# Exidekat/TransformerUpscaler

Hardware: AMD Instinct MI355X
Metric: images/sec, FastTransformer 2x 720p->1080p inference (higher is better)
Workload: dtype bf16

## Files before the change

transformerupscaler_amd/csrc/block_stream.hip:

```cpp
#include "common.h"
#include <stdlib.h>
#include <type_traits>
#include <utility>

namespace {

typedef __attribute__((ext_vector_type(16))) float f32x16;

constexpr int BS_NT = 512;
constexpr int TILE = 12288;
constexpr int L_TAB = 0;
constexpr int L_A = 8192, L_WQK = L_A, L_WV = L_A + 2 * TILE;
constexpr int L_B = L_A + 4 * TILE;
constexpr int L_KX = L_B, L_VX = L_B + 16384;
constexpr int L_OF = L_B + 32768;
constexpr int BS_LDS = L_OF + 65536;
constexpr int CHUNK = 2 * TILE;
static_assert(BS_LDS <= 163840, "LDS");
static_assert(L_A + 6 * CHUNK <= BS_LDS && L_A + 3 * CHUNK >= L_B + 2 * TILE, "MLP ring: six slots; slots 3-5 (the first chunks) clear of the proj tiles");
constexpr int T_QKB = 0, T_B1 = 384, T_BP = 1152, T_B2 = 1344;
constexpr int PROJ_T[6] = {L_WV, L_WQK, L_WV + TILE, L_WQK + TILE, L_B, L_B + TILE};

struct StreamBlock { const char* wqk; const char* wv; const char* wproj; const char* w1; const char* w2; const float* tab; const float* sbias; };
template <int PAR_, bool F1_, bool GE_, bool F2_, bool DM_> struct MlpSlot {
    static constexpr int PAR = PAR_, NM = (F1_ && F2_) ? 24 : 12;
    static constexpr bool F1 = F1_, GE = GE_, F2 = F2_, DM = DM_;
    static constexpr bool LNS = !F1_ && !GE_ && F2_;
};
constexpr int BS_MAX_BLK = 8;
struct StreamTable { StreamBlock b[BS_MAX_BLK]; };

template <class F, int... I> TUP_DEVICE void static_for_impl(F&& f, std::integer_sequence<int, I...>) { (f(std::integral_constant<int, I>{}), ...); }
template <int N, class F> TUP_DEVICE void static_for(F&& f) { static_for_impl(f, std::make_integer_sequence<int, N>{}); }

TUP_DEVICE f32x16 mfma32(bf16x8 a, bf16x8 b, f32x16 c) { return __builtin_amdgcn_mfma_f32_32x32x16_bf16(a, b, c, 0, 0, 0); }
TUP_DEVICE f32x16 mfma32h(bf16x8 a, bf16x8 b, f32x16 c) {
    return __builtin_amdgcn_mfma_f32_32x32x16_f16(__builtin_bit_cast(h8, a), __builtin_bit_cast(h8, b), c, 0, 0, 0);
}
#define FENCE() __builtin_amdgcn_sched_barrier(0)

TUP_DEVICE void lds_write_b128(uint32_t addr, bf16x8 v) { asm volatile("ds_write_b128 %0, %1" ::"v"(addr), "v"(v) : "memory"); }
TUP_DEVICE void lds_write_b128_off(uint32_t addr, bf16x8 v, int off) { asm volatile("ds_write_b128 %0, %1 offset:%2" ::"v"(addr), "v"(v), "i"(off) : "memory"); }
TUP_DEVICE void lds_write_b32(uint32_t addr, float v) { asm volatile("ds_write_b32 %0, %1" ::"v"(addr), "v"(v) : "memory"); }
TUP_DEVICE uint32_t lds_read_b32_off(uint32_t addr, int off) {
    uint32_t v;
    asm volatile("ds_read_b32 %0, %1 offset:%2" : "=v"(v) : "v"(addr), "i"(off));
    return v;
}
TUP_DEVICE f32x4 lds_read_f4_off(uint32_t addr, int off) { return __builtin_bit_cast(f32x4, lds_read_b128_asm_off(addr, off)); }
template <int N> TUP_DEVICE void vm_wait() { asm volatile("s_waitcnt vmcnt(%0)" ::"n"(N) : "memory"); }
TUP_DEVICE void barrier_all() {
    asm volatile("s_waitcnt vmcnt(0) lgkmcnt(0)\n\ts_barrier" ::: "memory");
}

TUP_DEVICE __amdgpu_buffer_rsrc_t bs_rsrc(const void* p) { return __builtin_amdgcn_make_buffer_rsrc(const_cast<void*>(p), 0, 0x7fffffff, 0x00020000); }
TUP_DEVICE void bs_dma(__amdgpu_buffer_rsrc_t r, char* lds_dst, uint32_t lane16, int soff) {
    __builtin_amdgcn_raw_ptr_buffer_load_lds(r, (__attribute__((address_space(3))) void*)lds_dst, 16, (int)lane16, soff, 0, 0);
}

#pragma clang diagnostic push
#pragma clang diagnostic ignored "-Winline-asm"
template <int OFF> TUP_DEVICE void bs_dma_on(__amdgpu_buffer_rsrc_t rs, uint32_t lds_base, uint32_t lane16, uint32_t soff) {
    static_assert(OFF >= 0 && OFF < 4096, "12-bit immediate offset");
    asm volatile("s_bitcmp1_b32 %0, 31\n\ts_cbranch_scc1 1f\n\ts_mov_b32 m0, %0\n\ts_nop 0\n\tbuffer_load_dwordx4 %1, %2, %3 offen offset:%4 lds\n1:"
                 :: "s"(lds_base), "v"(lane16), "s"(rs), "s"(soff), "n"(OFF) : "memory", "scc", "m0");
}
#pragma clang diagnostic pop

TUP_DEVICE bf16x8 pack8(float a0, float a1, float a2, float a3, float a4, float a5, float a6, float a7) {
    return __builtin_bit_cast(bf16x8, u32x4{pack_bf16x2(a0, a1), pack_bf16x2(a2, a3), pack_bf16x2(a4, a5), pack_bf16x2(a6, a7)});
}
template <int O> TUP_DEVICE bf16x8 pack8_regs(const f32x16& v) { return pack8(v[O], v[O + 1], v[O + 2], v[O + 3], v[O + 4], v[O + 5], v[O + 6], v[O + 7]); }
TUP_DEVICE float half_sum(float v) {
    const uint32_t u = __builtin_bit_cast(uint32_t, v);
    const auto q = __builtin_amdgcn_permlane32_swap(u, u, false, false);
    return __builtin_bit_cast(float, q[0]) + __builtin_bit_cast(float, opaque_copy(q[1]));
}
TUP_DEVICE float half_max(float v) {
    const uint32_t u = __builtin_bit_cast(uint32_t, v);
    const auto q = __builtin_amdgcn_permlane32_swap(u, u, false, false);
    return vmax(__builtin_bit_cast(float, q[0]), __builtin_bit_cast(float, opaque_copy(q[1])));
}
TUP_DEVICE float max3(float a, float b, float c) { return __builtin_fmaxf(__builtin_fmaxf(a, b), c); }

struct LnStats { float s[2], q[2]; };
TUP_DEVICE void ln_stats_tile(LnStats& st, const f32x16& t) {
#pragma unroll
    for (int i = 0; i < 16; ++i) { st.s[i & 1] += t[i]; st.q[i & 1] = __builtin_fmaf(t[i], t[i], st.q[i & 1]); }
}
template <int K> TUP_DEVICE void ln_stats_op(LnStats& st, const f32x16& t) {
    constexpr int i = K >> 1;
    if constexpr ((K & 1) == 0) { st.s[i & 1] += t[i]; asm volatile("" : "+v"(st.s[i & 1])); }
    else { st.q[i & 1] = __builtin_fmaf(t[i], t[i], st.q[i & 1]); asm volatile("" : "+v"(st.q[i & 1])); }
}
template <int K0, int K1> TUP_DEVICE void ln_stats_ops(LnStats& st, const f32x16& t) {
    static_for<(K1 > K0 ? K1 - K0 : 0)>([&](auto k) { ln_stats_op<K0 + decltype(k)::value>(st, t); });
}
TUP_DEVICE void ln_finish(const LnStats& st, float& rstd, float& shift) {
    const float sum = half_sum(st.s[0] + st.s[1]), sq = half_sum(st.q[0] + st.q[1]);
    const float mean = sum * (1.0f / 192);
    rstd = rsqrtf(fmaxf(__builtin_fmaf(-mean, mean, sq * (1.0f / 192)), 0.f) + 1e-5f);
    shift = -mean * rstd;
}
template <int U> TUP_DEVICE bf16x8 ln_frag(const f32x16& t, float rstd, float shift) {
    constexpr int O = 8 * U;
    return pack8(__builtin_fmaf(t[O], rstd, shift), __builtin_fmaf(t[O + 1], rstd, shift), __builtin_fmaf(t[O + 2], rstd, shift),
                 __builtin_fmaf(t[O + 3], rstd, shift), __builtin_fmaf(t[O + 4], rstd, shift), __builtin_fmaf(t[O + 5], rstd, shift),
                 __builtin_fmaf(t[O + 6], rstd, shift), __builtin_fmaf(t[O + 7], rstd, shift));
}

constexpr int SM_MAX_OPS = 20, SM_OPS = 56;
struct SmState { float c[4]; bf16x8 nmB; };
template <int K> TUP_DEVICE void softmax_op(SmState& st, f32x16 (&S)[2], bf16x8 (&P)[4], bool h0) {
    if constexpr (K < 16) {
        constexpr int ch = K & 3, step = K >> 2;
        constexpr int t = ch >> 1, o = 8 * (ch & 1);
        if constexpr (step == 0) st.c[ch] = max3(S[t][o], S[t][o + 1], S[t][o + 2]);
        else if constexpr (step == 1) st.c[ch] = max3(st.c[ch], S[t][o + 3], S[t][o + 4]);
        else if constexpr (step == 2) st.c[ch] = max3(st.c[ch], S[t][o + 5], S[t][o + 6]);
        else st.c[ch] = vmax(st.c[ch], S[t][o + 7]);
    } else if constexpr (K == 16) st.c[0] = max3(st.c[0], st.c[1], st.c[2]);
    else if constexpr (K == 17) st.c[0] = vmax(st.c[0], st.c[3]);
    else if constexpr (K == 18) st.c[0] = half_max(st.c[0]);
    else if constexpr (K == 19) {
        const uint32_t nm = pack_bf16x2(-st.c[0], 0.f);
        st.nmB = __builtin_bit_cast(bf16x8, u32x4{h0 ? nm : 0u, 0u, 0u, 0u});
    } else if constexpr (K < 52) {
        constexpr int k = K - 20, t = k >> 4, i = k & 15;
        S[t][i] = __builtin_amdgcn_exp2f(S[t][i]);
    } else {
        constexpr int f = K - 52;
        if constexpr ((f & 1) == 0) P[f] = pack8_regs<0>(S[f >> 1]); else P[f] = pack8_regs<8>(S[f >> 1]);
    }
}
template <int K0, int K1> TUP_DEVICE void softmax_ops(SmState& st, f32x16 (&S)[2], bf16x8 (&P)[4], bool h0) {
    static_for<(K1 > K0 ? K1 - K0 : 0)>([&](auto k) { softmax_op<K0 + decltype(k)::value>(st, S, P, h0); });
}

constexpr int GELU_OPS = 64;
struct GeluState { h2 x[4], sv[4], q[4]; };
#define TUP_PIN4(A) asm volatile("" : "+v"(A[3]))
template <int K> TUP_DEVICE void gelu_op(GeluState& g, const f32x16& acc, bf16x8 (&hf)[2]) {
    constexpr int b = K / 32, k = K % 32;
    if constexpr (k < 4) {
        g.x[k] = __builtin_convertvector(f32x2{acc[8 * b + 2 * k], acc[8 * b + 2 * k + 1]}, h2);
    } else {
        constexpr int t = (k - 4) >> 2, i = (k - 4) & 3;
        constexpr float C[3] = {0.82089258f, -0.67178146f, 0.70430058f};
        const h2 zero = {(_Float16)0.0f, (_Float16)0.0f}, one = {(_Float16)1.0f, (_Float16)1.0f};
        if constexpr (t == 0) g.sv[i] = __builtin_elementwise_fma(g.x[i], g.x[i], h2{(_Float16)-0.5f, (_Float16)-0.5f});
        else if constexpr (t == 1) g.q[i] = __builtin_elementwise_fma(g.sv[i], h2{(_Float16)2.74597983f, (_Float16)2.74597983f}, h2{(_Float16)-1.28256022f, (_Float16)-1.28256022f});
        else if constexpr (t < 5) g.q[i] = __builtin_elementwise_fma(g.q[i], g.sv[i], h2{(_Float16)C[t - 2], (_Float16)C[t - 2]});
        else if constexpr (t == 5) g.q[i] = __builtin_elementwise_min(__builtin_elementwise_max(__builtin_elementwise_fma(g.x[i], g.q[i], h2{(_Float16)0.5f, (_Float16)0.5f}), zero), one);
        else g.x[i] = g.x[i] * g.q[i];
    }
}
template <int K> TUP_DEVICE void gelu_pin(GeluState& g, bf16x8 (&hf)[2]) {
    constexpr int b = K / 32, k = K % 32;
    if constexpr (k >= 4 && ((k - 4) & 3) == 3) {
        constexpr int t = (k - 4) >> 2;
        if constexpr (t == 0) TUP_PIN4(g.sv);
        else if constexpr (t < 6) TUP_PIN4(g.q);
        else {
            TUP_PIN4(g.x);
            u32x4 pk;
#pragma unroll
            for (int n = 0; n < 4; ++n) pk[n] = __builtin_bit_cast(uint32_t, g.x[n]);
            hf[b] = __builtin_bit_cast(bf16x8, pk);
        }
    }
}
template <int K0, int K1> TUP_DEVICE void gelu_pins(GeluState& g, bf16x8 (&hf)[2]) {
    static_for<(K1 > K0 ? K1 - K0 : 0)>([&](auto k) { gelu_pin<K0 + decltype(k)::value>(g, hf); });
}
template <int K0, int K1> TUP_DEVICE void gelu_ops(GeluState& g, const f32x16& acc, bf16x8 (&hf)[2]) {
    static_for<(K1 > K0 ? K1 - K0 : 0)>([&](auto k) { gelu_op<K0 + decltype(k)::value>(g, acc, hf); });
}


constexpr int BS_NPH = 20;
enum { Q_PRO = 0, Q_BAR_PRO, Q_A0, Q_BAR_A0, Q_SLOT, Q_BAR_SLOT, Q_PROJ_PRE, Q_BAR_X, Q_PROJ, Q_LN2, Q_BAR_Y, Q_MLP, Q_BAR_MLP, Q_TOTAL, Q_S_DMA, Q_S_LOOP, Q_S_PV, Q_M_DMA };
__device__ unsigned long long tup_bs_stamps[2][8][BS_NPH];
TUP_DEVICE unsigned long long bs_now() {
    unsigned long long t;
    __builtin_amdgcn_sched_barrier(0);
    asm volatile("s_memtime %0\n\ts_waitcnt lgkmcnt(0)" : "=s"(t)::"memory");
    __builtin_amdgcn_sched_barrier(0);
    return t;
}

template <bool STAMPS>
__global__ __launch_bounds__(BS_NT, 2) void blocks_stream_kernel(float* __restrict__ xio, bf16_t* __restrict__ xout16, int nwin, const StreamTable tbl, int nblk)
{
    extern __shared__ __attribute__((aligned(16))) char smem[];
    const uint32_t sbase = lds_addr(smem);
    f32x16 R[6];
    bf16x8 tf[12];
    LnStats ln1{};
    unsigned long long ph[BS_NPH] = {}, tprev = 0, tstart = 0;
    if constexpr (STAMPS) tprev = tstart = bs_now();
#define BS_STAMP(K) do { if constexpr (STAMPS) { const unsigned long long t_ = bs_now(); ph[K] += t_ - tprev; tprev = t_; } } while (0)

#pragma unroll 1
    for (int blk = 0; blk < nblk; ++blk) {
    int tid = threadIdx.x;
    asm volatile("" : "+v"(tid));
    __builtin_assume(tid >= 0 && tid < BS_NT);
    const int lane = tid & 63, wave = __builtin_amdgcn_readfirstlane(tid >> 6);
    const int r = lane & 31, h = lane >> 5;
    const int hf = wave & 1;
    const int win = blockIdx.x * 4 + (wave >> 1);
    const bool active = win < nwin;
    const int row0 = (active ? win : nwin - 1) * 64 + 32 * hf;
    typedef __attribute__((address_space(1))) char* gptr_b;
    gptr_b xpark_b = (gptr_b)(xio + (size_t)row0 * 192);
    asm volatile("" : "+s"(xpark_b));
    const uint32_t lane16u = (uint32_t)lane * 16;
    struct { const char* wqk; const char* wv; const char* wproj; const char* wmlp; const float* tab; const float* sbias; } bp;
    {
        const StreamBlock& kb = tbl.b[blk];
        bp.wqk = kb.wqk; bp.wv = kb.wv; bp.wproj = kb.wproj; bp.wmlp = wave < 2 ? kb.w1 : kb.w2; bp.tab = kb.tab; bp.sbias = kb.sbias;
        asm volatile("" : "+s"(bp.wqk), "+s"(bp.wv), "+s"(bp.wproj), "+s"(bp.wmlp), "+s"(bp.tab), "+s"(bp.sbias));
    }
    const uint32_t lane16 = (uint32_t)lane * 16;
    uint32_t woff[4];
#pragma unroll
    for (int t = 0; t < 4; ++t) woff[t] = sbase + (uint32_t)(r * 128 + (((2 * t + h) ^ ((r >> 1) & 7)) << 4));
    const uint32_t tabh = sbase + L_TAB + (uint32_t)h * 64;
    const uint32_t tabr = sbase + L_TAB + (uint32_t)r * 4;
    const uint32_t kx_wr = sbase + L_KX + (uint32_t)wave * 1024 + lane16, kx_rd = sbase + L_KX + (uint32_t)(wave ^ 1) * 1024 + lane16;
    const uint32_t vx_wr = sbase + L_VX + (uint32_t)wave * 2048 + lane16, vx_rd = sbase + L_VX + (uint32_t)(wave ^ 1) * 2048 + lane16;
    const uint32_t of_ad = sbase + L_OF + (uint32_t)wave * 8192 + lane16;
    const bf16x8 onesB = __builtin_bit_cast(bf16x8, u32x4{h == 0 ? 0x3f803f80u : 0u, 0u, 0u, 0u});
    const bf16x8 onesA = __builtin_bit_cast(bf16x8, u32x4{h == 0 ? 0x00003f80u : 0u, 0u, 0u, 0u});

    auto dma_tile_piece = [&](const char* src, int tile, int lds_off, int half, int u) {
        (void)half;
        if (wave < 4) { const int pc = wave * 3 + u; bs_dma(bs_rsrc(src), smem + lds_off + pc * 1024, lane16, tile * TILE + pc * 1024); }
    };
    auto dma_tile = [&](const char* src, int tile, int lds_off, int half) {
        if ((wave >> 2) == half) {
            const __amdgpu_buffer_rsrc_t rs = bs_rsrc(src);
#pragma unroll
            for (int u = 0; u < 3; ++u) { const int pc = (wave & 3) * 3 + u; bs_dma(rs, smem + lds_off + pc * 1024, lane16, tile * TILE + pc * 1024); }
        }
    };

    if (blk == 0) {
        const float* xg = xio + (size_t)(row0 + (lane >> 3)) * 192 + 4 * (lane & 7);
        char* scr = smem + L_OF + wave * 8192;
        f32x4 tmp[6][4];
#pragma unroll
        for (int rt = 0; rt < 6; ++rt)
#pragma unroll
            for (int j = 0; j < 4; ++j) tmp[rt][j] = *reinterpret_cast<const f32x4*>(xg + (size_t)(8 * j) * 192 + 32 * rt);
#pragma unroll
        for (int rt = 0; rt < 6; ++rt) {
#pragma unroll
            for (int j = 0; j < 4; ++j) *reinterpret_cast<f32x4*>(scr + j * 1024 + lane * 16) = tmp[rt][j];
#pragma unroll
            for (int m = 0; m < 4; ++m) {
                const f32x4 v = *reinterpret_cast<const f32x4*>(scr + r * 128 + (4 * h + m) * 16);
#pragma unroll
                for (int e = 0; e < 4; ++e) R[rt][4 * m + e] = v[e];
            }
        }
    }
    typedef const __attribute__((address_space(1))) float* gptr_f;
    typedef const __attribute__((address_space(1))) f32x4* gptr_f4;
    const gptr_f tabg = (gptr_f)bp.tab;
    const float tb0 = tabg[tid], tb1 = tabg[512 + tid], tb2 = tabg[1024 + tid];
    __syncthreads();
    {
        const uint32_t ta = sbase + L_TAB + (uint32_t)tid * 4;
        lds_write_b32(ta, tb0); lds_write_b32(ta + 2048, tb1); lds_write_b32(ta + 4096, tb2);
    }
    FENCE();
    dma_tile(bp.wqk, 0, L_WQK, 0);
    dma_tile(bp.wv, 0, L_WV, 1);
    dma_tile(bp.wqk, 1, L_WQK + TILE, 0);
    dma_tile(bp.wv, 1, L_WV + TILE, 1);
    float ln_rstd, ln_shift;
    {
        if (blk == 0) {
            ln1 = LnStats{};
#pragma unroll
            for (int rt = 0; rt < 4; ++rt) ln_stats_tile(ln1, R[rt]);
        }
        ln_stats_tile(ln1, R[4]); ln_stats_tile(ln1, R[5]);
        ln_finish(ln1, ln_rstd, ln_shift);
        tf[0] = ln_frag<0>(R[0], ln_rstd, ln_shift);
        ln1 = LnStats{};
    }
    FENCE();

    f32x16 accqk, accv, S[2], O;
    bf16x8 Qf, Kfo, Kfp, Vfo[2], Vfp[2], P[4], Ofr[4];
    typedef const __attribute__((address_space(1))) char* gptr_c;
    const uint32_t lane64u = (uint32_t)lane * 64;
    auto load_sbias = [&](int hd) {
#pragma unroll
        for (int t = 0; t < 2; ++t) {
            const int kt = t == 0 ? hf : 1 - hf;
            gptr_c sb = (gptr_c)bp.sbias + (size_t)(((hd * 2 + hf) * 2 + kt) * 4096);
            asm volatile("" : "+s"(sb));
            const gptr_f4 p4 = (gptr_f4)(sb + lane64u);
#pragma unroll
            for (int m = 0; m < 4; ++m) {
                const f32x4 v = p4[m];
#pragma unroll
                for (int e = 0; e < 4; ++e) S[t][4 * m + e] = v[e];
            }
        }
    };
#define WFRAG(T, s) lds_read_b128_asm_off(woff[(s) & 3], (T) + ((s) >> 2) * 4096)
#define BIASQ(OFF, m) lds_read_f4_off(tabh, ((OFF) + 4 * (m)) * 4)
    auto acc_from4 = [](f32x4 a, f32x4 b, f32x4 c, f32x4 d) {
        return f32x16{a[0], a[1], a[2], a[3], b[0], b[1], b[2], b[3], c[0], c[1], c[2], c[3], d[0], d[1], d[2], d[3]};
    };
    const f32x16 zero16 = {0.f, 0.f, 0.f, 0.f, 0.f, 0.f, 0.f, 0.f, 0.f, 0.f, 0.f, 0.f, 0.f, 0.f, 0.f, 0.f};

    load_sbias(0);
    BS_STAMP(Q_PRO);
    barrier_all();
    BS_STAMP(Q_BAR_PRO);
    {
        const f32x4 b0 = BIASQ(T_QKB + 0, 0), b1 = BIASQ(T_QKB + 0, 1), b2 = BIASQ(T_QKB + 0, 2), b3 = BIASQ(T_QKB + 0, 3);
        bf16x8 wq[4];
        wq[0] = WFRAG(L_WQK, 0); wq[1] = WFRAG(L_WQK, 1); wq[2] = WFRAG(L_WQK, 2);
        lds_wait<3>();
        FENCE();
        accqk = acc_from4(b0, b1, b2, b3);
        accv = zero16;
        static_for<24>([&](auto g_) {
            constexpr int g = decltype(g_)::value;
            if constexpr (g + 3 < 24) {
                if constexpr (g + 3 < 12) wq[(g + 3) & 3] = WFRAG(L_WQK, g + 3); else wq[(g + 3) & 3] = WFRAG(L_WV, g + 3 - 12);
                lds_wait<3>();
            } else lds_wait<23 - g>();
            FENCE();
            if constexpr (g < 12) accqk = mfma32(wq[g & 3], tf[g], accqk);
            else accv = mfma32(tf[g - 12], wq[g & 3], accv);
            if constexpr (g + 1 < 12) tf[g + 1] = ln_frag<(g + 1) & 1>(R[(g + 1) >> 1], ln_rstd, ln_shift);
            {
                constexpr int rt = g >> 2, m = g & 3;
                gptr_b pb = xpark_b + rt * 4096;
                asm volatile("" : "+s"(pb));
                if (active) *(__attribute__((address_space(1))) f32x4*)(pb + m * 1024 + lane16u) = f32x4{R[rt][4 * m], R[rt][4 * m + 1], R[rt][4 * m + 2], R[rt][4 * m + 3]};
            }
            FENCE();
        });
        Qf = pack8_regs<0>(accqk); Kfo = pack8_regs<8>(accqk);
        Vfo[0] = pack8_regs<0>(accv); Vfo[1] = pack8_regs<8>(accv);
        lds_write_b128(kx_wr, Kfo);
        lds_write_b128(vx_wr, Vfo[0]); lds_write_b128_off(vx_wr, Vfo[1], 1024);
        FENCE();
        BS_STAMP(Q_A0);
        barrier_all();
        BS_STAMP(Q_BAR_A0);
    }

    static_for<12>([&](auto hd_) {
        constexpr int hd = decltype(hd_)::value;
        constexpr int NQK = hd + 1 < 12 ? 12 : 0;
        constexpr int VP = hd / 2 + 1;
        constexpr int NV = VP < 6 ? 6 : 0, V0 = (hd & 1) * 6;
        constexpr int NG = NQK + NV;
        constexpr int TQK = L_WQK + ((hd + 1) & 1) * TILE, TV = L_WV + (VP & 1) * TILE;
        constexpr bool DQK = hd + 2 < 12, DV = (hd & 1) == 0 && hd / 2 + 2 < 6;
        constexpr int PJ0 = hd == 8 ? 0 : hd == 10 ? 1 : hd == 11 ? 3 : -1, PJ1 = hd == 10 ? 2 : -1;
        Kfp = lds_read_b128_asm_off(kx_rd, (hd & 1) * 8192);
        if constexpr ((hd & 1) == 0) { Vfp[0] = lds_read_b128_asm_off(vx_rd, 0); Vfp[1] = lds_read_b128_asm_off(vx_rd, 1024); }
        lds_wait<0>();
        FENCE();
        BS_STAMP(Q_S_DMA);
        constexpr int GS = -1;
        if constexpr (GS < 0) { S[0] = mfma32(Kfo, Qf, S[0]); S[1] = mfma32(Kfp, Qf, S[1]); FENCE(); }
        SmState sm;
        if constexpr (NG > 0) {
            const f32x4 b0 = BIASQ(T_QKB + (hd + 1) * 32, 0), b1 = BIASQ(T_QKB + (hd + 1) * 32, 1), b2 = BIASQ(T_QKB + (hd + 1) * 32, 2),
                        b3 = BIASQ(T_QKB + (hd + 1) * 32, 3);
            bf16x8 wq[4];
            auto frag = [&](auto g_) {
                constexpr int g = decltype(g_)::value;
                if constexpr (g < NQK) return WFRAG(TQK, g); else return WFRAG(TV, V0 + g - NQK);
            };
            wq[0] = frag(std::integral_constant<int, 0>{}); wq[1] = frag(std::integral_constant<int, 1>{}); wq[2] = frag(std::integral_constant<int, 2>{});
            lds_wait<2>();
            FENCE();
            if constexpr (NQK > 0) accqk = acc_from4(b0, b1, b2, b3);
            if constexpr (NV > 0 && V0 == 0) accv = zero16;
            static_for<NG>([&](auto g_) {
                constexpr int g = decltype(g_)::value;
                if constexpr (g < NQK) accqk = mfma32(wq[g & 3], tf[g], accqk);
                else accv = mfma32(tf[V0 + g - NQK], wq[g & 3], accv);
                if constexpr (g == 1 || g == 4 || g == 7) {
                    if constexpr (DQK) dma_tile_piece(bp.wqk, hd + 2, L_WQK + (hd & 1) * TILE, hd & 1, g / 3);
                    if constexpr (DV) dma_tile_piece(bp.wv, hd / 2 + 2, L_WV + ((hd / 2) & 1) * TILE, 1 - (hd & 1), g / 3);
                    if constexpr (PJ0 >= 0) dma_tile_piece(bp.wproj, PJ0, PROJ_T[PJ0], PJ0 & 1, g / 3);
                    if constexpr (PJ1 >= 0) dma_tile_piece(bp.wproj, PJ1, PROJ_T[PJ1], PJ1 & 1, g / 3);
                }
                if constexpr (g == GS) { S[0] = mfma32(Kfo, Qf, S[0]); S[1] = mfma32(Kfp, Qf, S[1]); }
                constexpr int G0 = GS + 3, GM = G0 + 4, GE = GM + 3, NGV = NG - GE;
                if constexpr (g >= G0 && g < GM) softmax_ops<(SM_MAX_OPS * (g - G0)) / 4, (SM_MAX_OPS * (g - G0 + 1)) / 4>(sm, S, P, h == 0);
                if constexpr (g == GM) { S[0] = mfma32(onesA, sm.nmB, S[0]); S[1] = mfma32(onesA, sm.nmB, S[1]); }
                if constexpr (g >= GE) softmax_ops<SM_MAX_OPS + ((SM_OPS - SM_MAX_OPS) * (g - GE)) / NGV, SM_MAX_OPS + ((SM_OPS - SM_MAX_OPS) * (g - GE + 1)) / NGV>(sm, S, P, h == 0);
                if constexpr (g + 3 < NG) wq[(g + 3) & 3] = frag(std::integral_constant<int, g + 3>{});
                if constexpr (g + 1 < NG) lds_wait<(NG - 2 - g < 2 ? NG - 2 - g : 2)>();
                FENCE();
            });
        } else {
            if constexpr (PJ0 >= 0) dma_tile(bp.wproj, PJ0, PROJ_T[PJ0], PJ0 & 1);
            softmax_ops<0, SM_MAX_OPS>(sm, S, P, h == 0);
            FENCE();
            S[0] = mfma32(onesA, sm.nmB, S[0]); S[1] = mfma32(onesA, sm.nmB, S[1]);
            FENCE();
            softmax_ops<SM_MAX_OPS, SM_OPS>(sm, S, P, h == 0);
            FENCE();
        }
        BS_STAMP(Q_S_LOOP);
        if constexpr (hd + 1 < 12) load_sbias(hd + 1);
        FENCE();
        {
            const bool mine = (hd & 1) == 0 ? r < 16 : r >= 16;
            auto sel = [&](bf16x8 v) {
                const u32x4 u = __builtin_bit_cast(u32x4, v);
                return __builtin_bit_cast(bf16x8, u32x4{mine ? u[0] : 0x3f803f80u, mine ? u[1] : 0x3f803f80u, mine ? u[2] : 0x3f803f80u, mine ? u[3] : 0x3f803f80u});
            };
            const bf16x8 v0 = sel(Vfo[0]), v1 = sel(Vfo[1]);
            FENCE();
            O = mfma32(v0, P[0], zero16);
            O = mfma32(v1, P[1], O);
            const bf16x8 v2 = sel(Vfp[0]), v3 = sel(Vfp[1]);
            FENCE();
            O = mfma32(v2, P[2], O);
            O = mfma32(v3, P[3], O);
            FENCE();
        }
        BS_STAMP(Q_S_PV);
        if constexpr (NQK > 0) {
            Qf = pack8_regs<0>(accqk); Kfo = pack8_regs<8>(accqk);
            lds_write_b128_off(kx_wr, Kfo, ((hd + 1) & 1) * 8192);
        }
        if constexpr (NV > 0 && V0 == 6) {
            Vfo[0] = pack8_regs<0>(accv); Vfo[1] = pack8_regs<8>(accv);
            lds_write_b128(vx_wr, Vfo[0]); lds_write_b128_off(vx_wr, Vfo[1], 1024);
        }
        FENCE();
        {
            constexpr int c0 = (hd & 1) == 0 ? 0 : 8, s0 = (hd & 1) == 0 ? 8 : 0;
            const float inv = __builtin_amdgcn_rcpf(O[s0]);
            const bf16x8 of = pack8(O[c0] * inv, O[c0 + 1] * inv, O[c0 + 2] * inv, O[c0 + 3] * inv, O[c0 + 4] * inv, O[c0 + 5] * inv,
                                    O[c0 + 6] * inv, O[c0 + 7] * inv);
            if constexpr (hd < 8) lds_write_b128_off(of_ad, of, hd * 1024); else Ofr[hd - 8] = of;
        }
        FENCE();
        BS_STAMP(Q_SLOT);
        if constexpr (hd + 1 < 12) asm volatile("s_waitcnt vmcnt(8) lgkmcnt(0)\n\ts_barrier" ::: "memory");
        else barrier_all();
        BS_STAMP(Q_BAR_SLOT);
    });

    dma_tile(bp.wproj, 4, PROJ_T[4], 0);
    dma_tile(bp.wproj, 5, PROJ_T[5], 1);
    bf16x8 Ofl[8];
#pragma unroll
    for (int i = 0; i < 8; ++i) Ofl[i] = lds_read_b128_asm_off(of_ad, i * 1024);
    auto load_park = [&](auto rt_, auto m_) {
        constexpr int rt = decltype(rt_)::value, m = decltype(m_)::value;
        gptr_b pb = xpark_b + rt * 4096;
        asm volatile("" : "+s"(pb));
        const f32x4 v = *(const __attribute__((address_space(1))) f32x4*)(pb + m * 1024 + lane16u);
#pragma unroll
        for (int e = 0; e < 4; ++e) R[rt][4 * m + e] = v[e];
    };
    static_for<8>([&](auto i_) { load_park(std::integral_constant<int, decltype(i_)::value / 4>{}, std::integral_constant<int, decltype(i_)::value % 4>{}); });
    lds_wait<0>();
    FENCE();
    BS_STAMP(Q_PROJ_PRE);
    const int mw = wave * 6;
    auto dma_chunk_piece = [&](int c, int lds_off, int u) {
        if (wave < 4) { const int pc = mw + u; bs_dma(bs_rsrc(bp.wmlp), smem + lds_off + pc * 1024, lane16, c * TILE + (wave < 2 ? pc : pc - 12) * 1024); }
    };
    const __amdgpu_buffer_rsrc_t rs_mlp = bs_rsrc(bp.wmlp);
    const uint32_t mlp_lds0 = __builtin_amdgcn_readfirstlane(sbase + (uint32_t)(mw * 1024) + (wave < 4 ? 0u : 0x80000000u));
    const uint32_t mlp_src0 = __builtin_amdgcn_readfirstlane((uint32_t)((wave < 2 ? mw : mw - 12) * 1024));
    auto dma_chunk = [&](int c, int lds_off) {
#pragma unroll
        for (int u = 0; u < 6; ++u) dma_chunk_piece(c, lds_off, u);
    };
    auto ring_off = [&](int c) { return L_A + ((c + 3) % 6) * CHUNK; };
    {
        LnStats st{};
        static_for<6>([&](auto rt_) {
            constexpr int rt = decltype(rt_)::value;
            if constexpr (rt == 4) {
                BS_STAMP(Q_PROJ);
                barrier_all();
                BS_STAMP(Q_BAR_X);
                dma_chunk(0, ring_off(0));
                dma_chunk(1, ring_off(1));
            }
            constexpr int TB = rt < 4 ? 0 : L_B, T = PROJ_T[rt] - TB;
            uint32_t wb[4];
#pragma unroll
            for (int t = 0; t < 4; ++t) wb[t] = woff[t] + TB;
#define WFRAGB(T, s) lds_read_b128_asm_off(wb[(s) & 3], (T) + ((s) >> 2) * 4096)
            bf16x8 wq[4];
            wq[0] = WFRAGB(T, 0); wq[1] = WFRAGB(T, 1); wq[2] = WFRAGB(T, 2);
            const uint32_t bw = lds_read_b32_off(tabr, (T_BP + rt * 32) * 4);
            lds_wait<0>();
            FENCE();
            static_for<12>([&](auto g_) {
                constexpr int g = decltype(g_)::value;
                if constexpr (g + 3 < 12) { wq[(g + 3) & 3] = WFRAGB(T, g + 3); lds_wait<3>(); } else lds_wait<11 - g>();
                FENCE();
                if constexpr (g < 8) R[rt] = mfma32(wq[g & 3], Ofl[g], R[rt]); else R[rt] = mfma32(wq[g & 3], Ofr[g - 8], R[rt]);
                if constexpr (rt + 2 < 6 && g % 3 == 1) load_park(std::integral_constant<int, rt + 2>{}, std::integral_constant<int, g / 3>{});
                if constexpr (rt > 0 && g >= 3) ln_stats_ops<(32 * (g - 3)) / 9, (32 * (g - 2)) / 9>(st, R[rt - 1]);
                FENCE();
            });
            R[rt] = mfma32(__builtin_bit_cast(bf16x8, u32x4{bw, 0u, 0u, 0u}), onesB, R[rt]);
            FENCE();
        });
        BS_STAMP(Q_PROJ);
        ln_stats_tile(st, R[5]);
        float rstd, shift;
        ln_finish(st, rstd, shift);
#pragma unroll
        for (int rt = 0; rt < 6; ++rt) { tf[2 * rt] = ln_frag<0>(R[rt], rstd, shift); tf[2 * rt + 1] = ln_frag<1>(R[rt], rstd, shift); }
        static_for<6>([&](auto rt_) {
            constexpr int rt = decltype(rt_)::value;
            const uint32_t bw = lds_read_b32_off(tabr, (T_B2 + rt * 32) * 4);
            lds_wait<0>();
            FENCE();
            R[rt] = mfma32(__builtin_bit_cast(bf16x8, u32x4{bw, 0u, 0u, 0u}), onesB, R[rt]);
        });
    }
    FENCE();
    BS_STAMP(Q_LN2);
    barrier_all();
    BS_STAMP(Q_BAR_Y);

    {
        f32x16 acc1[2];
        bf16x8 hfr[2][2];
        GeluState gs;
        uint32_t w2off[2];
#pragma unroll
        for (int u = 0; u < 2; ++u) w2off[u] = sbase + (uint32_t)(r * 64 + (((2 * u + h) ^ ((r >> 2) & 3)) << 4));
        int ri = 3;
        auto pair = [&](auto A_, auto B_, int c) {
            using A = decltype(A_); using B = decltype(B_);
            static_assert(!B::DM && A::PAR == 0 && B::PAR == 1, "");
            constexpr int NA = A::NM, NB = B::NM, NT = NA + NB;
            auto wrap = [](int v) { return v >= 6 ? v - 6 : v; };
            uint32_t dl[2] = {0, 0}, ds[2] = {0, 0};
            if constexpr (A::DM) {
                dl[0] = mlp_lds0 + (uint32_t)(L_A + wrap(ri + 2) * CHUNK); dl[1] = mlp_lds0 + (uint32_t)(L_A + wrap(ri + 3) * CHUNK);
                ds[0] = mlp_src0 + (uint32_t)((c + 2) * TILE); ds[1] = ds[0] + TILE;
            }
            uint32_t a1[2][4], a2[2][2];
            {
                const uint32_t o1[2] = {(uint32_t)(L_A + ri * CHUNK), (uint32_t)(L_A + wrap(ri + 1) * CHUNK)};
                const uint32_t o2[2] = {(uint32_t)(L_A + wrap(ri + 4) * CHUNK + TILE), (uint32_t)(L_A + wrap(ri + 5) * CHUNK + TILE)};
#pragma unroll
                for (int q = 0; q < 2; ++q) {
#pragma unroll
                    for (int t = 0; t < 4; ++t) a1[q][t] = woff[t] + o1[q];
#pragma unroll
                    for (int u = 0; u < 2; ++u) a2[q][u] = w2off[u] + o2[q];
                }
            }
            ri = wrap(ri + 2);
            const uint32_t tb = tabh + (uint32_t)((T_B1 + c * 32) * 4);
            BS_STAMP(Q_M_DMA);
            auto frag = [&](auto g_) {
                constexpr int g = decltype(g_)::value, q = g < NA ? 0 : 1, n = g < NA ? g : g - NA;
                constexpr bool F1 = q == 0 ? A::F1 : B::F1, F2 = q == 0 ? A::F2 : B::F2;
                constexpr bool is1 = F1 && (!F2 || (n & 1) == 0);
                constexpr int k = (F1 && F2) ? n / 2 : n;
#ifdef TUP_BSX_NOLDS
                return __builtin_bit_cast(bf16x8, u32x4{a1[q][k & 3], a2[q][k & 1], (uint32_t)n, 0u});
#else
                if constexpr (is1) return lds_read_b128_asm_off(a1[q][k & 3], (k >> 2) * 4096);
                else return lds_read_b128_asm_off(a2[q][k & 1], (k >> 1) * 2048);
#endif
            };
            constexpr int LA = 5, RS = LA + 1;
            constexpr int NBIAS = A::GE ? (35 * NA) / GELU_OPS + 1 : 1;
            static_assert(!B::F1 || NBIAS + LA + 2 < NA, "the bias has landed before the second slot starts");
            bf16x8 wq[RS];
            f32x4 b0, b1, b2, b3, c0, c1, c2, c3;
            if constexpr (A::F1) { b0 = lds_read_f4_off(tb, 0); b1 = lds_read_f4_off(tb, 16); b2 = lds_read_f4_off(tb, 32); b3 = lds_read_f4_off(tb, 48); }
            static_for<LA>([&](auto i_) { wq[decltype(i_)::value] = frag(i_); });
            lds_wait<LA - 1>();
            FENCE();
            if constexpr (A::F1) acc1[0] = acc_from4(b0, b1, b2, b3);
            static_for<NT>([&](auto g_) {
                constexpr int g = decltype(g_)::value, q = g < NA ? 0 : 1, n = g < NA ? g : g - NA;
                constexpr int NM = q == 0 ? NA : NB, PAR = q;
                constexpr bool F1 = q == 0 ? A::F1 : B::F1, F2 = q == 0 ? A::F2 : B::F2, GE = q == 0 ? A::GE : B::GE;
                constexpr bool DM = q == 0 && A::DM, LNS = q == 0 ? A::LNS : B::LNS;
                constexpr bool is1 = F1 && (!F2 || (n & 1) == 0);
                constexpr int k = (F1 && F2) ? n / 2 : n;
                if constexpr (g == NA && B::F1) acc1[1] = acc_from4(c0, c1, c2, c3);
                if constexpr (is1) acc1[PAR] = mfma32(wq[g % RS], tf[k], acc1[PAR]);
                else R[k >> 1] = mfma32h(wq[g % RS], hfr[PAR][k & 1], R[k >> 1]);
                FENCE();
#ifndef TUP_BSX_NOGELU
                if constexpr (GE && n > 0) gelu_pins<(GELU_OPS * (n - 1)) / NM, (GELU_OPS * n) / NM>(gs, hfr[1 - PAR]);
#endif
                if constexpr (g + LA < NT) wq[(g + LA) % RS] = frag(std::integral_constant<int, g + LA>{});
                if constexpr (B::F1 && g == NBIAS) {
                    c0 = lds_read_f4_off(tb, 128); c1 = lds_read_f4_off(tb, 128 + 16); c2 = lds_read_f4_off(tb, 128 + 32); c3 = lds_read_f4_off(tb, 128 + 48);
                }
                if constexpr ((g & 1) == 0 && g + 1 < NT) {
                    constexpr int FR = NT - 3 - g < LA - 2 ? (NT - 3 - g < 0 ? 0 : NT - 3 - g) : LA - 2;
                    constexpr int BI = (B::F1 && g + 2 - LA <= NBIAS && NBIAS <= g) ? 4 : 0;
                    lds_wait<FR + BI>();
                }
#ifndef TUP_BSX_NOGELU
                if constexpr (GE) gelu_ops<(GELU_OPS * n) / NM, (GELU_OPS * (n + 1)) / NM>(gs, acc1[1 - PAR], hfr[1 - PAR]);
#else
                if constexpr (GE && n == NM - 1) { asm volatile("" :: "v"(acc1[1 - PAR])); asm volatile("" : "+v"(hfr[1 - PAR][0]), "+v"(hfr[1 - PAR][1])); }
#endif
#ifndef TUP_BSX_NODMA
                if constexpr (DM && n % (NM / 12) == NM / 12 - 1) {
                    constexpr int pi = n / (NM / 12);
                    constexpr int dq = pi / 6, u = pi % 6;
                    bs_dma_on<(u & 3) * 1024>(rs_mlp, dl[dq] + (u >> 2) * 4096, lane16, ds[dq] + (u >> 2) * 4096);
                }
#endif
                if constexpr (LNS && n >= 4) ln_stats_ops<16 * (n & 1), 16 * (n & 1) + 16>(ln1, R[(n - 4) >> 1]);
#ifndef TUP_BSX_NOGELU
                if constexpr (GE && n == NM - 1) gelu_pins<(GELU_OPS * n) / NM, GELU_OPS>(gs, hfr[1 - PAR]);
#endif
                FENCE();
            });
            BS_STAMP(Q_MLP);
        };
        auto pair_end = [&]() { barrier_all(); BS_STAMP(Q_BAR_MLP); };
        pair(MlpSlot<0, true, false, false, true>{}, MlpSlot<1, true, true, false, false>{}, 0);
        pair_end();
#pragma unroll 1
        for (int c = 2; c < 22; c += 2) {
            pair(MlpSlot<0, true, true, true, true>{}, MlpSlot<1, true, true, true, false>{}, c);
            pair_end();
        }
        pair(MlpSlot<0, true, true, true, false>{}, MlpSlot<1, true, true, true, false>{}, 22);
        pair(MlpSlot<0, false, true, true, false>{}, MlpSlot<1, false, false, true, false>{}, 24);
        BS_STAMP(Q_MLP);
    }
    }
    if (xout16 != nullptr) {
        int tid = threadIdx.x;
        asm volatile("" : "+v"(tid));
        const int lane = tid & 63, wave = tid >> 6, r = lane & 31, h = lane >> 5;
        const int win = blockIdx.x * 4 + (wave >> 1);
        char* scr = smem + L_OF + wave * 8192;
        char* og = reinterpret_cast<char*>(xout16) + (size_t)((win < nwin ? win : nwin - 1) * 64 + 32 * (wave & 1)) * 384;
#pragma unroll
        for (int q = 0; q < 2; ++q) {
#pragma unroll
            for (int t = 0; t < 3; ++t) {
                const f32x16& a = R[3 * q + t];
                *reinterpret_cast<bf16x8*>(scr + r * 192 + t * 64 + h * 32) = pack8(a[0], a[1], a[2], a[3], a[4], a[5], a[6], a[7]);
                *reinterpret_cast<bf16x8*>(scr + r * 192 + t * 64 + h * 32 + 16) = pack8(a[8], a[9], a[10], a[11], a[12], a[13], a[14], a[15]);
            }
#pragma unroll
            for (int j = 0; j < 6; ++j) {
                const int b = j * 1024 + lane * 16, row = b / 192, col = b - row * 192;
                const u32x4 v = *reinterpret_cast<const u32x4*>(scr + b);
                if (win < nwin) *reinterpret_cast<u32x4*>(og + (size_t)row * 384 + q * 192 + col) = v;
            }
        }
    } else {
        int tid = threadIdx.x;
        asm volatile("" : "+v"(tid));
        const int lane = tid & 63, wave = tid >> 6, r = lane & 31, h = lane >> 5;
        const int win = blockIdx.x * 4 + (wave >> 1);
        char* scr = smem + L_OF + wave * 8192;
        float* xg = xio + (size_t)((win < nwin ? win : nwin - 1) * 64 + 32 * (wave & 1) + (lane >> 3)) * 192 + 4 * (lane & 7);
#pragma unroll
        for (int rt = 0; rt < 6; ++rt) {
#pragma unroll
            for (int m = 0; m < 4; ++m)
                *reinterpret_cast<f32x4*>(scr + r * 128 + (4 * h + m) * 16) = f32x4{R[rt][4 * m], R[rt][4 * m + 1], R[rt][4 * m + 2], R[rt][4 * m + 3]};
#pragma unroll
            for (int j = 0; j < 4; ++j) {
                const f32x4 v = *reinterpret_cast<const f32x4*>(scr + j * 1024 + lane * 16);
                if (win < nwin) *reinterpret_cast<f32x4*>(xg + (size_t)(8 * j) * 192 + 32 * rt) = v;
            }
        }
    }
    if constexpr (STAMPS) {
        ph[Q_TOTAL] = bs_now() - tstart;
        const int b = blockIdx.x, rec = b == 0 ? 0 : (b == 300 ? 1 : -1);
        if (rec >= 0 && (threadIdx.x & 63) == 0)
#pragma unroll
            for (int k = 0; k < BS_NPH; ++k) tup_bs_stamps[rec][threadIdx.x >> 6][k] = ph[k];
    }
#undef BS_STAMP
#undef WFRAG
#undef WFRAGB
#undef BIASQ
}

}

extern "C" int tup_blocks_stream_fwd(float* x, void* out_bf16, const void* const* table, int nblk, int nwin, void* stream)
{
    if (nwin <= 0 || nblk <= 0) return 0;
    if (nblk > BS_MAX_BLK || table == nullptr) return (int)hipErrorInvalidValue;
    StreamTable t{};
    for (int i = 0; i < nblk; ++i) {
        const void* const* r = table + (size_t)i * 7;
        t.b[i] = StreamBlock{(const char*)r[0], (const char*)r[1], (const char*)r[2], (const char*)r[3], (const char*)r[4],
                             (const float*)r[5], (const float*)r[6]};
    }
    const int nwg = (nwin + 3) / 4;
#ifdef TUP_DIAG
    if (getenv("TUP_BS_STAMPS")) {
        TUP_SET_DYN_LDS(blocks_stream_kernel<true>, BS_LDS);
        blocks_stream_kernel<true><<<dim3(nwg), dim3(BS_NT), BS_LDS, reinterpret_cast<hipStream_t>(stream)>>>(x, reinterpret_cast<bf16_t*>(out_bf16), nwin, t, nblk);
        TUP_CHECK_LAUNCH();
        return 0;
    }
#endif
    TUP_SET_DYN_LDS(blocks_stream_kernel<false>, BS_LDS);
    blocks_stream_kernel<false><<<dim3(nwg), dim3(BS_NT), BS_LDS, reinterpret_cast<hipStream_t>(stream)>>>(x, reinterpret_cast<bf16_t*>(out_bf16), nwin, t, nblk);
    TUP_CHECK_LAUNCH();
    return 0;
}

#ifdef TUP_DIAG
extern "C" int tup_debug_bs_stamps(unsigned long long* host_out)
{
    return (int)hipMemcpyFromSymbol(host_out, HIP_SYMBOL(tup_bs_stamps), sizeof(unsigned long long) * 2 * 8 * BS_NPH);
}
#endif
```

Before: 2755.

## Prefetch next block's QK/V weights, bias table and sbias during final MLP pair

```diff
diff --git a/transformerupscaler_amd/csrc/block_stream.hip b/transformerupscaler_amd/csrc/block_stream.hip
--- a/transformerupscaler_amd/csrc/block_stream.hip
+++ b/transformerupscaler_amd/csrc/block_stream.hip
@@ -14,10 +14,11 @@
 constexpr int L_B = L_A + 4 * TILE;
 constexpr int L_KX = L_B, L_VX = L_B + 16384;
 constexpr int L_OF = L_B + 32768;
-constexpr int BS_LDS = L_OF + 65536;
+constexpr int L_TAB2 = L_OF + 65536;
+constexpr int BS_LDS = L_TAB2 + 6144;
 constexpr int CHUNK = 2 * TILE;
 static_assert(BS_LDS <= 163840, "LDS");
-static_assert(L_A + 6 * CHUNK <= BS_LDS && L_A + 3 * CHUNK >= L_B + 2 * TILE, "MLP ring: six slots; slots 3-5 (the first chunks) clear of the proj tiles");
+static_assert(L_A + 6 * CHUNK <= L_TAB2 && L_A + 3 * CHUNK >= L_B + 2 * TILE, "MLP ring: six slots; slots 3-5 (the first chunks) clear of the proj tiles");
 constexpr int T_QKB = 0, T_B1 = 384, T_BP = 1152, T_B2 = 1344;
 constexpr int PROJ_T[6] = {L_WV, L_WQK, L_WV + TILE, L_WQK + TILE, L_B, L_B + TILE};
 
@@ -27,6 +28,7 @@
     static constexpr bool F1 = F1_, GE = GE_, F2 = F2_, DM = DM_;
     static constexpr bool LNS = !F1_ && !GE_ && F2_;
 };
+constexpr int NX_PIECES = 9;
 constexpr int BS_MAX_BLK = 8;
 struct StreamTable { StreamBlock b[BS_MAX_BLK]; };
 
@@ -195,6 +197,7 @@
     extern __shared__ __attribute__((aligned(16))) char smem[];
     const uint32_t sbase = lds_addr(smem);
     f32x16 R[6];
+    f32x16 S[2];
     bf16x8 tf[12];
     LnStats ln1{};
     unsigned long long ph[BS_NPH] = {}, tprev = 0, tstart = 0;
@@ -226,8 +229,9 @@
     uint32_t woff[4];
 #pragma unroll
     for (int t = 0; t < 4; ++t) woff[t] = sbase + (uint32_t)(r * 128 + (((2 * t + h) ^ ((r >> 1) & 7)) << 4));
-    const uint32_t tabh = sbase + L_TAB + (uint32_t)h * 64;
-    const uint32_t tabr = sbase + L_TAB + (uint32_t)r * 4;
+    const uint32_t tab_img = sbase + (uint32_t)((blk & 1) ? L_TAB2 : L_TAB);
+    const uint32_t tabh = tab_img + (uint32_t)h * 64;
+    const uint32_t tabr = tab_img + (uint32_t)r * 4;
     const uint32_t kx_wr = sbase + L_KX + (uint32_t)wave * 1024 + lane16, kx_rd = sbase + L_KX + (uint32_t)(wave ^ 1) * 1024 + lane16;
     const uint32_t vx_wr = sbase + L_VX + (uint32_t)wave * 2048 + lane16, vx_rd = sbase + L_VX + (uint32_t)(wave ^ 1) * 2048 + lane16;
     const uint32_t of_ad = sbase + L_OF + (uint32_t)wave * 8192 + lane16;
@@ -268,18 +272,35 @@
     }
     typedef const __attribute__((address_space(1))) float* gptr_f;
     typedef const __attribute__((address_space(1))) f32x4* gptr_f4;
-    const gptr_f tabg = (gptr_f)bp.tab;
-    const float tb0 = tabg[tid], tb1 = tabg[512 + tid], tb2 = tabg[1024 + tid];
-    __syncthreads();
-    {
-        const uint32_t ta = sbase + L_TAB + (uint32_t)tid * 4;
+    typedef const __attribute__((address_space(1))) char* gptr_c;
+    const uint32_t lane64u = (uint32_t)lane * 64;
+    auto load_sbias_of = [&](const float* sbias, int hd) {
+#pragma unroll
+        for (int t = 0; t < 2; ++t) {
+            const int kt = t == 0 ? hf : 1 - hf;
+            gptr_c sb = (gptr_c)sbias + (size_t)(((hd * 2 + hf) * 2 + kt) * 4096);
+            asm volatile("" : "+s"(sb));
+            const gptr_f4 p4 = (gptr_f4)(sb + lane64u);
+#pragma unroll
+            for (int m = 0; m < 4; ++m) {
+                const f32x4 v = p4[m];
+#pragma unroll
+                for (int e = 0; e < 4; ++e) S[t][4 * m + e] = v[e];
+            }
+        }
+    };
+    auto load_sbias = [&](int hd) { load_sbias_of(bp.sbias, hd); };
+    if (blk == 0) {
+        const gptr_f tabg = (gptr_f)bp.tab;
+        const float tb0 = tabg[tid], tb1 = tabg[512 + tid], tb2 = tabg[1024 + tid];
+        const uint32_t ta = tab_img + (uint32_t)tid * 4;
         lds_write_b32(ta, tb0); lds_write_b32(ta + 2048, tb1); lds_write_b32(ta + 4096, tb2);
-    }
-    FENCE();
-    dma_tile(bp.wqk, 0, L_WQK, 0);
-    dma_tile(bp.wv, 0, L_WV, 1);
-    dma_tile(bp.wqk, 1, L_WQK + TILE, 0);
-    dma_tile(bp.wv, 1, L_WV + TILE, 1);
+        FENCE();
+        dma_tile(bp.wqk, 0, L_WQK, 0);
+        dma_tile(bp.wv, 0, L_WV, 1);
+        dma_tile(bp.wqk, 1, L_WQK + TILE, 0);
+        load_sbias(0);
+    }
     float ln_rstd, ln_shift;
     {
         if (blk == 0) {
@@ -294,25 +315,8 @@
     }
     FENCE();
 
-    f32x16 accqk, accv, S[2], O;
+    f32x16 accqk, accv, O;
     bf16x8 Qf, Kfo, Kfp, Vfo[2], Vfp[2], P[4], Ofr[4];
-    typedef const __attribute__((address_space(1))) char* gptr_c;
-    const uint32_t lane64u = (uint32_t)lane * 64;
-    auto load_sbias = [&](int hd) {
-#pragma unroll
-        for (int t = 0; t < 2; ++t) {
-            const int kt = t == 0 ? hf : 1 - hf;
-            gptr_c sb = (gptr_c)bp.sbias + (size_t)(((hd * 2 + hf) * 2 + kt) * 4096);
-            asm volatile("" : "+s"(sb));
-            const gptr_f4 p4 = (gptr_f4)(sb + lane64u);
-#pragma unroll
-            for (int m = 0; m < 4; ++m) {
-                const f32x4 v = p4[m];
-#pragma unroll
-                for (int e = 0; e < 4; ++e) S[t][4 * m + e] = v[e];
-            }
-        }
-    };
 #define WFRAG(T, s) lds_read_b128_asm_off(woff[(s) & 3], (T) + ((s) >> 2) * 4096)
 #define BIASQ(OFF, m) lds_read_f4_off(tabh, ((OFF) + 4 * (m)) * 4)
     auto acc_from4 = [](f32x4 a, f32x4 b, f32x4 c, f32x4 d) {
@@ -320,10 +324,10 @@
     };
     const f32x16 zero16 = {0.f, 0.f, 0.f, 0.f, 0.f, 0.f, 0.f, 0.f, 0.f, 0.f, 0.f, 0.f, 0.f, 0.f, 0.f, 0.f};
 
-    load_sbias(0);
     BS_STAMP(Q_PRO);
     barrier_all();
     BS_STAMP(Q_BAR_PRO);
+    dma_tile(bp.wv, 1, L_WV + TILE, 1);
     {
         const f32x4 b0 = BIASQ(T_QKB + 0, 0), b1 = BIASQ(T_QKB + 0, 1), b2 = BIASQ(T_QKB + 0, 2), b3 = BIASQ(T_QKB + 0, 3);
         bf16x8 wq[4];
@@ -550,6 +554,9 @@
 #pragma unroll
         for (int u = 0; u < 2; ++u) w2off[u] = sbase + (uint32_t)(r * 64 + (((2 * u + h) ^ ((r >> 2) & 3)) << 4));
         int ri = 3;
+        const char* nx_wqk = nullptr; const char* nx_wv = nullptr;
+        uint32_t nx_lds0 = 0x80000000u;
+        const uint32_t nx_src0 = __builtin_amdgcn_readfirstlane((uint32_t)(wave * 3 * 1024));
         auto pair = [&](auto A_, auto B_, int c) {
             using A = decltype(A_); using B = decltype(B_);
             static_assert(!B::DM && A::PAR == 0 && B::PAR == 1, "");
@@ -631,6 +638,11 @@
                     constexpr int dq = pi / 6, u = pi % 6;
                     bs_dma_on<(u & 3) * 1024>(rs_mlp, dl[dq] + (u >> 2) * 4096, lane16, ds[dq] + (u >> 2) * 4096);
                 }
+                if constexpr (!A::F1 && (g & 1) == 1 && g < 2 * NX_PIECES) {
+                    constexpr int j = (g >> 1) / 3, u = (g >> 1) % 3;
+                    bs_dma_on<u * 1024>(bs_rsrc(j < 2 ? nx_wqk : nx_wv), nx_lds0 + (uint32_t)(j == 0 ? L_WQK : j == 1 ? L_WQK + TILE : L_WV), lane16,
+                                        nx_src0 + (uint32_t)(j == 1 ? TILE : 0));
+                }
 #endif
                 if constexpr (LNS && n >= 4) ln_stats_ops<16 * (n & 1), 16 * (n & 1) + 16>(ln1, R[(n - 4) >> 1]);
 #ifndef TUP_BSX_NOGELU
@@ -649,8 +661,24 @@
             pair_end();
         }
         pair(MlpSlot<0, true, true, true, false>{}, MlpSlot<1, true, true, true, false>{}, 22);
+        pair_end();
+        const bool more = blk + 1 < nblk;
+        const float* nx_tab; const float* nx_sbias;
+        {
+            const StreamBlock& kn = tbl.b[more ? blk + 1 : blk];
+            nx_wqk = kn.wqk; nx_wv = kn.wv; nx_tab = kn.tab; nx_sbias = kn.sbias;
+            asm volatile("" : "+s"(nx_wqk), "+s"(nx_wv), "+s"(nx_tab), "+s"(nx_sbias));
+        }
+        nx_lds0 = __builtin_amdgcn_readfirstlane(sbase + (uint32_t)(wave * 3 * 1024) + (wave < 4 && more ? 0u : 0x80000000u));
+        const gptr_f tabn = (gptr_f)nx_tab;
+        const float tn0 = tabn[tid], tn1 = tabn[512 + tid], tn2 = tabn[1024 + tid];
+        load_sbias_of(nx_sbias, 0);
         pair(MlpSlot<0, false, true, true, false>{}, MlpSlot<1, false, false, true, false>{}, 24);
         BS_STAMP(Q_MLP);
+        {
+            const uint32_t ta = sbase + (uint32_t)((blk & 1) ? L_TAB : L_TAB2) + (uint32_t)tid * 4;
+            lds_write_b32(ta, tn0); lds_write_b32(ta + 2048, tn1); lds_write_b32(ta + 4096, tn2);
+        }
     }
     }
     if (xout16 != nullptr) {
```

Result: no change. 2763 (median of 6 runs) (+0.3%).
